# BraveenSri/siddhi

Hardware: AMD Instinct MI355X
Metric: events/sec (whole node) for partitioned pattern query at 1/2/4/8 GPUs; % HBM peak (higher is better)
Workload: dtype f32

## Files before the change

### siddhi_amd/csrc/gwalk.h

```cpp
#pragma once
#include <hip/hip_runtime.h>

#include <algorithm>
#include <cstdlib>
#include <cstring>
#include <type_traits>

#include "keypart.h"
#include "sg_engine.h"
#include "sg_prim.h"
#include "walk.h"

struct GwArgs {
  int64_t n, nc;
  int64_t within;
  int64_t t0;
  uint32_t K, ns1;
  int32_t stack_mode;
  int32_t cap;
  int32_t chunk;
  int32_t carry_out;
  int32_t pzero;
  const uint32_t* o1;
  const PtU4* grec;
  const uint8_t* glk;
  const uint32_t* kbase;
  uint64_t* trig;
  uint64_t* area;
  int64_t* cv_ts;
  int32_t* cv_key;
  int64_t* cv_val;
  int64_t* cv_pay;
  uint32_t* cv_n;
  uint32_t cv_cap;
  uint32_t* flags;
  uint32_t* ovf_keys;
  uint32_t* ovf_n;
  uint32_t ovf_cap;
  uint32_t* match_n;
};
static const uint32_t GW_ORDER = 1, GW_OVERFLOW = 2, GW_INTERNAL = 4, GW_CARRY_FULL = 8;

static __global__ void __launch_bounds__(256) k_gw_count(const uint32_t* __restrict__ o1, uint32_t ns1, uint32_t K,
                                                         const uint8_t* __restrict__ glk, uint32_t* __restrict__ kcnt) {
  __shared__ uint32_t c[4][256];
  const uint32_t g = blockIdx.x, t = threadIdx.x, w = t >> 6;
#pragma unroll
  for (int q = 0; q < 4; ++q) c[q][t] = 0;
  __syncthreads();
  const uint32_t lo = o1[(size_t)g * ns1], hi = o1[(size_t)(g + 1) * ns1];
  for (uint32_t p = lo + t; p < hi; p += 256) atomicAdd(&c[w][glk[p]], 1u);
  __syncthreads();
  const uint32_t k = (g << 8) + t;
  if (k < K) kcnt[k] = c[0][t] + c[1][t] + c[2][t] + c[3][t];
}

template <int PT>
struct GwLds {
  PtU4 stage[256 * PT];
  uint32_t cw[4][256];
  uint32_t ls[256], tot[256];
  uint32_t wsum[4];
};

template <class T>
struct GwLdsRing {
  T* v;
  int32_t* t;
  int32_t* p;
  uint32_t cmask, lane;
  __device__ __forceinline__ uint32_t ix(uint32_t s) const { return (s & cmask) * 256 + lane; }
  __device__ __forceinline__ bool full(uint32_t head, uint32_t top) const { return top - head == cmask + 1; }
};
template <class T>
struct GwHbmRing {
  T* v;
  int32_t* t;
  int32_t* p;
  __device__ __forceinline__ uint32_t ix(uint32_t s) const { return s; }
  __device__ __forceinline__ bool full(uint32_t, uint32_t) const { return false; }
};

template <class T, int OP, bool STACK, class RING>
struct GwLane {
  RING R;
  uint32_t head = 0, top = 0;
  int32_t hts = 0, prev = INT32_MIN;
  T tv = T();
  bool bad = false;
  uint64_t cur = 0;
  uint32_t k = 0;
  uint32_t nm = 0;
  uint32_t wi = 0;
  __device__ __forceinline__ bool step(const GwArgs& a, const PtU4& q) {
    const int32_t dts = (int32_t)q.x;
    const uint32_t rowf = q.y;
    T x;
    const uint32_t xb = q.z;
    __builtin_memcpy(&x, &xb, sizeof(T));
    const int32_t pay = (int32_t)q.w;
    const uint32_t f = rowf >> 30;
    bad |= dts < prev;
    prev = dts;
    if (!f) return true;
    const bool live = !is_nan_val<T>(x);
    if (head != top && (uint32_t)(dts - hts) > wi) {
      ++head;
      while (head != top) {
        hts = R.t[R.ix(head)];
        if ((uint32_t)(dts - hts) <= wi) break;
        ++head;
      }
    }
    const uint32_t r = rowf & ROW_MASK;
    uint32_t m = 0;
    if ((f & F_CONS) && live) {
      const bool emit = r >= (uint32_t)a.nc;
      const uint64_t hdr = cur;
      if constexpr (STACK) {
        if (top != head && cmp_op<T>(OP, x, tv)) {
          --top;
          ++m;
          while (top != head) {
            tv = R.v[R.ix(top - 1)];
            if (!cmp_op<T>(OP, x, tv)) break;
            --top;
            ++m;
          }
        }
        if (emit && m) {
          for (uint32_t e = 0; e < m; ++e) {
            const uint32_t s = R.ix(top + e);
            a.area[hdr + 2 + e] = (uint64_t)(uint32_t)val_bits<T>(R.v[s]) | ((uint64_t)(uint32_t)R.p[s] << 32);
          }
        }
      } else {
        uint32_t wr = head;
        for (uint32_t s = head; s != top; ++s) {
          const uint32_t si = R.ix(s);
          const T e = R.v[si];
          if (cmp_op<T>(OP, x, e)) {
            if (emit) a.area[hdr + 2 + m] = (uint64_t)(uint32_t)val_bits<T>(e) | ((uint64_t)(uint32_t)R.p[si] << 32);
            ++m;
          } else {
            if (wr != s) {
              const uint32_t wx = R.ix(wr);
              R.v[wx] = e;
              R.t[wx] = R.t[si];
              R.p[wx] = R.p[si];
            }
            ++wr;
          }
        }
        top = wr;
        if (head != top) {
          hts = R.t[R.ix(head)];
          tv = R.v[R.ix(top - 1)];
        }
      }
      if (emit && m) {
        const uint64_t b = r - (uint32_t)a.nc;
        a.area[hdr] = (uint64_t)(uint32_t)dts | ((uint64_t)k << 32);
        a.area[hdr + 1] = (uint64_t)(uint32_t)val_bits<T>(x) | ((uint64_t)(uint32_t)pay << 32);
        a.trig[b] = hdr | ((uint64_t)m << 32);
        cur = hdr + 2 + m;
        nm += m;
      }
    }
    if ((f & F_CAND) && live) {
      if (R.full(head, top)) return false;
      const uint32_t s = R.ix(top);
      R.v[s] = x;
      R.t[s] = dts;
      R.p[s] = pay;
      if (top == head) hts = dts;
      tv = x;
      ++top;
    }
    return true;
  }
  __device__ __forceinline__ void carry(const GwArgs& a, uint32_t o) const {
    for (uint32_t e = 0; e < top - head; ++e) {
      const uint32_t s = R.ix(head + e);
      a.cv_ts[o + e] = a.t0 + (int64_t)R.t[s];
      a.cv_key[o + e] = (int32_t)k;
      a.cv_val[o + e] = val_bits<T>(R.v[s]);
      a.cv_pay[o + e] = a.pzero ? (int64_t)(uint32_t)R.p[s] : (int64_t)R.p[s];
    }
  }
};

template <class T, int OP, int PT, bool STACK>
__global__ void __launch_bounds__(256, 1) k_gwalk(GwArgs a) {
  extern __shared__ __attribute__((aligned(16))) char lds_raw[];
  GwLds<PT>& L = *(GwLds<PT>*)lds_raw;
  const uint32_t cap = (uint32_t)a.cap;
  const uint32_t t = threadIdx.x, w = t >> 6, lane = t & 63;
  const uint32_t g = xcd_block(blockIdx.x, gridDim.x);
  const uint32_t k = (g << 8) + t;
  const bool active = k < a.K;
  const uint32_t lo = a.o1[(size_t)g * a.ns1], hi = a.o1[(size_t)(g + 1) * a.ns1];
  GwLane<T, OP, STACK, GwLdsRing<T>> W;
  W.R.v = (T*)(lds_raw + sizeof(GwLds<PT>));
  W.R.t = (int32_t*)(W.R.v + (size_t)cap * 256);
  W.R.p = W.R.t + (size_t)cap * 256;
  W.R.cmask = cap - 1;
  W.R.lane = t;
  W.k = k;
  W.wi = a.within > 0xffffffffll ? 0xffffffffu : (uint32_t)a.within;
  W.cur = active ? 3ull * a.kbase[k] : 0ull;
  bool ovf = false;
  const uint32_t ROWS = 256 * PT;
  PtU4 rc[PT], rn[PT];
  uint32_t tg[PT], tn[PT];
  auto load = [&](uint32_t base, PtU4* r, uint32_t* d) {
    const uint32_t rows = min(ROWS, hi - base);
#pragma unroll
    for (int s = 0; s < PT; ++s) {
      const uint32_t i = w * (PT * 64) + s * 64 + lane;
      const uint32_t p = base + (i < rows ? i : rows - 1);
      r[s] = __builtin_nontemporal_load(a.grec + p);
      d[s] = a.glk[p];
    }
  };
  if (lo < hi) load(lo, rc, tg);
  for (uint32_t base = lo; base < hi; base += ROWS) {
    {
      const uint32_t rows = min(ROWS, hi - base);
#pragma unroll
      for (int s = 0; s < PT; ++s)
        if (w * (PT * 64) + s * 64 + lane >= rows) tg[s] = 0xffffffffu;
    }
#pragma unroll
    for (int q = 0; q < 4; ++q) L.cw[q][t] = 0;
    __syncthreads();
#pragma unroll
    for (int s = 0; s < PT; ++s)
      if (tg[s] != 0xffffffffu) atomicAdd(&L.cw[w][tg[s]], 1u);
    __syncthreads();
    {
      const uint32_t c0 = L.cw[0][t], c1 = L.cw[1][t], c2 = L.cw[2][t], c3 = L.cw[3][t];
      const uint32_t tt = c0 + c1 + c2 + c3;
      const uint32_t ex = block_excl_scan256(tt, L.wsum);
      L.ls[t] = ex;
      L.tot[t] = tt;
      L.cw[0][t] = ex;
      L.cw[1][t] = ex + c0;
      L.cw[2][t] = ex + c0 + c1;
      L.cw[3][t] = ex + c0 + c1 + c2;
    }
    __syncthreads();
#pragma unroll
    for (int s = 0; s < PT; ++s) {
      const bool valid = tg[s] != 0xffffffffu;
      const uint32_t d = valid ? tg[s] : 0u;
      uint32_t rank, cnt;
      peer_rank(valid, d, 8, rank, cnt);
      if (valid) {
        const uint32_t slot = L.cw[w][d] + rank;
        if (rank == 0) L.cw[w][d] = slot + cnt;
        L.stage[slot] = rc[s];
      }
    }
    if (base + ROWS < hi) load(base + ROWS, rn, tn);
    __syncthreads();
    const uint32_t i0 = L.ls[t], i1 = i0 + L.tot[t];
    for (uint32_t i = i0; i < i1 && active && !ovf; ++i)
      if (!W.step(a, L.stage[i])) ovf = true;
    __syncthreads();
#pragma unroll
    for (int s = 0; s < PT; ++s) { rc[s] = rn[s]; tg[s] = tn[s]; }
  }
  uint32_t fl = W.bad ? GW_ORDER : 0u;
  if (active && W.cur > 3ull * a.kbase[k + 1]) fl |= GW_INTERNAL;
  if (ovf) {
    const uint32_t o = atomicAdd(a.ovf_n, 1u);
    if (o < a.ovf_cap) a.ovf_keys[o] = k;
    else fl |= GW_OVERFLOW;
  }
  if (fl) atomicOr(a.flags, fl);
  {
    uint32_t c = (active && !ovf) ? W.nm : 0u;
#pragma unroll
    for (int o = 32; o > 0; o >>= 1) c += (uint32_t)__shfl_xor((int)c, o);
    if (lane == 0 && c) atomicAdd(a.match_n, c);
  }
  if (!a.carry_out) return;
  const uint32_t m = (active && !ovf) ? W.top - W.head : 0u;
  uint32_t incl = m;
#pragma unroll
  for (int o = 1; o < 64; o <<= 1) {
    const uint32_t y = (uint32_t)__shfl_up((int)incl, o);
    if ((int)lane >= o) incl += y;
  }
  const uint32_t tot = (uint32_t)__shfl((int)incl, 63);
  if (!tot) return;
  uint32_t cb = 0;
  if (lane == 63) cb = atomicAdd(a.cv_n, tot);
  cb = (uint32_t)__shfl((int)cb, 63);
  if ((uint64_t)cb + tot > (uint64_t)a.cv_cap) {
    if (lane == 63) atomicOr(a.flags, GW_CARRY_FULL);
    return;
  }
  if (m) W.carry(a, cb + incl - m);
}

static const uint32_t GW_REDO_LDS = 2048;
template <class T, int OP, bool STACK>
__global__ void __launch_bounds__(256) k_gw_redo(GwArgs a, uint32_t* __restrict__ rows, T* __restrict__ hv,
                                                 int32_t* __restrict__ ht, int32_t* __restrict__ hp) {
  __shared__ uint32_t wc[4], base_s;
  __shared__ PtU4 red_stage[GW_REDO_LDS];
  __shared__ T red_v[GW_REDO_LDS];
  __shared__ int32_t red_t[GW_REDO_LDS], red_p[GW_REDO_LDS];
  const uint32_t k = a.ovf_keys[blockIdx.x];
  const uint32_t g = k >> 8, d = k & 255u, t = threadIdx.x, w = t >> 6, lane = t & 63;
  const uint32_t lo = a.o1[(size_t)g * a.ns1], hi = a.o1[(size_t)(g + 1) * a.ns1];
  const uint32_t kb = a.kbase[k], ke = a.kbase[k + 1];
  if (t == 0) base_s = 0;
  __syncthreads();
  for (uint32_t p0 = lo; p0 < hi; p0 += 256) {
    const uint32_t p = p0 + t;
    const bool mine = p < hi && a.glk[p] == d;
    const uint64_t bm = __ballot(mine);
    const uint32_t below = __builtin_amdgcn_mbcnt_hi((uint32_t)(bm >> 32), __builtin_amdgcn_mbcnt_lo((uint32_t)bm, 0u));
    if (lane == 0) wc[w] = (uint32_t)__popcll(bm);
    __syncthreads();
    uint32_t before = base_s;
    for (uint32_t q = 0; q < w; ++q) before += wc[q];
    if (mine && kb + before + below < ke) rows[kb + before + below] = p;
    __syncthreads();
    if (t == 0) base_s += wc[0] + wc[1] + wc[2] + wc[3];
    __syncthreads();
  }
  const uint32_t nk = ke - kb;
  const bool in_lds = nk <= GW_REDO_LDS;
  if (in_lds)
    for (uint32_t i = t; i < nk; i += 256) red_stage[i] = a.grec[rows[kb + i]];
  __syncthreads();
  if (t != 0) return;
  if (kb + base_s != ke) { atomicOr(a.flags, GW_INTERNAL); return; }
  GwLane<T, OP, STACK, GwHbmRing<T>> W;
  if (in_lds) {
    W.R.v = red_v;
    W.R.t = red_t;
    W.R.p = red_p;
  } else {
    W.R.v = hv + kb;
    W.R.t = ht + kb;
    W.R.p = hp + kb;
  }
  W.k = k;
  W.wi = a.within > 0xffffffffll ? 0xffffffffu : (uint32_t)a.within;
  W.cur = 3ull * kb;
  if (in_lds) for (uint32_t i = 0; i < nk; ++i) W.step(a, red_stage[i]);
  else for (uint32_t i = kb; i < ke; ++i) W.step(a, a.grec[rows[i]]);
  uint32_t fl = W.bad ? GW_ORDER : 0u;
  if (W.cur > 3ull * ke) fl |= GW_INTERNAL;
  if (fl) atomicOr(a.flags, fl);
  if (W.nm) atomicAdd(a.match_n, W.nm);
  if (!a.carry_out) return;
  const uint32_t m = W.top - W.head;
  if (!m) return;
  const uint32_t o = atomicAdd(a.cv_n, m);
  if ((uint64_t)o + m > (uint64_t)a.cv_cap) { atomicOr(a.flags, GW_CARRY_FULL); return; }
  W.carry(a, o);
}

struct GwSel {
  int32_t n_select, stride, multi, b_slot, pzero, vfloat;
  int32_t code[SG_MAX_SELECT];
};
static const int GW_PROJ_S = 256;
static const int GW_TILE = 256;

static __global__ void __launch_bounds__(256) k_gtile_count(int64_t n, const uint64_t* __restrict__ trig,
                                                            uint32_t* __restrict__ tcount, int64_t ntile) {
  __shared__ uint32_t red[8][4];
  const uint32_t t = threadIdx.x, w = t >> 6, lane = t & 63;
#pragma unroll
  for (int s = 0; s < 8; ++s) {
    const int64_t r = ((int64_t)blockIdx.x * 8 + s) * GW_TILE + t;
    uint32_t c = r < n ? (uint32_t)(__builtin_nontemporal_load(trig + r) >> 32) : 0u;
#pragma unroll
    for (int o = 32; o > 0; o >>= 1) c += (uint32_t)__shfl_xor((int)c, o);
    if (lane == 0) red[s][w] = c;
  }
  __syncthreads();
  if (t < 8) {
    const int64_t tile = (int64_t)blockIdx.x * 8 + t;
    if (tile < ntile) tcount[tile] = red[t][0] + red[t][1] + red[t][2] + red[t][3];
  }
}

static __global__ void __launch_bounds__(256) k_gscan_project(int64_t n, int64_t t0, uint64_t base_index,
                                                              const uint64_t* __restrict__ index,
                                                              const uint64_t* __restrict__ trig,
                                                              const uint64_t* __restrict__ area, GwSel sel,
                                                              int64_t out_base, char* __restrict__ out,
                                                              const uint32_t* __restrict__ tbase) {
  extern __shared__ __attribute__((aligned(16))) char stage[];
  __shared__ uint32_t wsum[4];
  const uint32_t t = threadIdx.x;
  const int64_t b = (int64_t)blockIdx.x * GW_TILE + t;
  const uint64_t tw = b < n ? __builtin_nontemporal_load(trig + b) : 0ull;
  const uint32_t m = (uint32_t)(tw >> 32);
  const uint64_t u = (uint32_t)tw;
  uint64_t h0 = 0, h1 = 0, tg = 0;
  if (m) {
    h0 = area[u];
    h1 = area[u + 1];
    tg = index ? index[b] : base_index + (uint64_t)b;
  }
  const uint32_t excl = block_excl_scan256(m, wsum);
  const uint32_t pre = tbase[blockIdx.x];
  const uint32_t o_lo = pre, o_hi = pre + (wsum[0] + wsum[1] + wsum[2] + wsum[3]);
  const uint32_t o = pre + excl;
  auto wid = [&](uint32_t bits, bool zero) { return zero ? (int64_t)bits : (int64_t)(int32_t)bits; };
  uint32_t nmask = 0;
  for (int s = 0; s < sel.n_select; ++s) nmask |= (sel.code[s] == 4) ? 1u << s : 0u;
  const int64_t ts = t0 + (int64_t)(int32_t)(uint32_t)h0;
  const uint32_t key = (uint32_t)(h0 >> 32);
  const int64_t v2 = wid((uint32_t)h1, sel.vfloat), p2 = wid((uint32_t)(h1 >> 32), sel.pzero);
  typedef uint32_t U4 __attribute__((ext_vector_type(4)));
  for (uint32_t sub = o_lo; sub < o_hi; sub += GW_PROJ_S) {
    const uint32_t se = (o_hi - sub < (uint32_t)GW_PROJ_S) ? o_hi : sub + GW_PROJ_S;
    if (m && o < se && o + m > sub) {
      const uint32_t qa = o < sub ? sub - o : 0u, qe = (o + m > se) ? se - o : m;
      for (uint32_t q = qa; q < qe; ++q) {
        const uint64_t e = area[u + 2 + q];
        const int64_t v1 = wid((uint32_t)e, sel.vfloat), p1 = wid((uint32_t)(e >> 32), sel.pzero);
        int64_t* r = (int64_t*)(stage + (size_t)(o + q - sub) * sel.stride);
        r[0] = (int64_t)tg;
        r[1] = ts;
        r[2] = (int64_t)((uint64_t)key | ((uint64_t)((1u << 24) | (sel.multi ? (uint32_t)sel.b_slot : (0x800000u | q))) << 32));
        r[3] = (int64_t)nmask;
        for (int c = 0; c < sel.n_select; ++c) {
          const int code = sel.code[c];
          r[4 + c] = code == 0 ? p1 : code == 1 ? v1 : code == 2 ? v2 : code == 3 ? p2 : 0;
        }
      }
    }
    __syncthreads();
    const size_t bytes = (size_t)(se - sub) * sel.stride;
    char* dst = out + (size_t)(out_base + sub) * sel.stride;
    if ((((uintptr_t)dst) & 15) == 0) {
      for (size_t x = (size_t)t * 16; x + 16 <= bytes; x += 256 * 16) *(U4*)(dst + x) = *(const U4*)(stage + x);
      if ((bytes & 8) && t == 255) *(uint64_t*)(dst + bytes - 8) = *(const uint64_t*)(stage + bytes - 8);
    } else {
      for (size_t x = (size_t)t * 8; x < bytes; x += 256 * 8) *(uint64_t*)(dst + x) = *(const uint64_t*)(stage + x);
    }
    __syncthreads();
  }
}

struct GwPlan {
  bool ok = false;
  int cap = 0;
  GwSel sel;
};
template <class T>
static GwPlan gw_plan(SgHandle* h, const BatchView& bv, int64_t n, int64_t nc, uint32_t kb, const PushPlan& plan,
                      bool same_col, int64_t span_ms) {
  const sg_nfa_desc& d = h->desc;
  GwPlan g;
  memset(&g.sel, 0, sizeof(g.sel));
  if (!d.partitioned || !same_col || plan.e1_row || d.n_select > SG_MAX_SELECT) return g;
  for (int c = 0; c < d.n_cols; ++c)
    if (bv.cols.nul[c]) return g;
  for (int s = 0; s < d.n_select; ++s) {
    const int src = plan.pp.src[s], kind = plan.pp.kind[s];
    int code = -1;
    if (kind == 2) code = 4;
    else if (kind == 0 && src == 0) code = 0;
    else if (kind == 1) code = src ? 2 : 1;
    else if (kind == 3 && src == 1 && plan.pcol >= 0 && plan.pp.col[s] == plan.pcol) code = 3;
    if (code < 0) return g;
    g.sel.code[s] = code;
  }
  const int64_t win = window_rows(kb, nc + n, d.within, span_ms);
  const char* e = getenv("SG_DEBUG_GW_CAP");
  int cap = h->opt.ring_cap > 0 ? h->opt.ring_cap : (e ? atoi(e) : pick_cap(win));
  if (cap > 32 || cap < 2 || (cap & (cap - 1))) return g;
  g.cap = cap;
  g.sel.n_select = d.n_select;
  g.sel.stride = 32 + 8 * d.n_select;
  g.sel.vfloat = std::is_same<T, float>::value ? 1 : 0;
  g.ok = true;
  return g;
}

template <class T, int OP, int PT, bool STACK>
static void launch_gwalk_pt(const GwArgs& ga, uint32_t ng, hipStream_t st) {
  const size_t lds = sizeof(GwLds<PT>) + (size_t)ga.cap * 256 * (sizeof(T) + 8);
  HIPCHK(hipFuncSetAttribute((const void*)k_gwalk<T, OP, PT, STACK>, hipFuncAttributeMaxDynamicSharedMemorySize, (int)lds));
  hipLaunchKernelGGL((k_gwalk<T, OP, PT, STACK>), dim3(ng), dim3(256), lds, st, ga);
  HIPCHK(hipGetLastError());
}
template <class T, int OP>
static void launch_gw_redo(const GwArgs& ga, uint32_t nk, uint32_t* rows, T* hv, int32_t* ht, int32_t* hp, hipStream_t st) {
  if (ga.stack_mode) hipLaunchKernelGGL((k_gw_redo<T, OP, true>), dim3(nk), dim3(256), 0, st, ga, rows, hv, ht, hp);
  else hipLaunchKernelGGL((k_gw_redo<T, OP, false>), dim3(nk), dim3(256), 0, st, ga, rows, hv, ht, hp);
  HIPCHK(hipGetLastError());
}
template <class T, int OP>
static void launch_gwalk(const GwArgs& ga, uint32_t ng, hipStream_t st) {
  const char* e = getenv("SG_DEBUG_GW_PT");
  const int pt = e ? atoi(e) : (ga.cap <= 8 ? 8 : ga.cap <= 16 ? 6 : 4);
  if (ga.stack_mode) {
    if (pt == 4) launch_gwalk_pt<T, OP, 4, true>(ga, ng, st);
    else if (pt == 12) launch_gwalk_pt<T, OP, 12, true>(ga, ng, st);
    else if (pt == 10) launch_gwalk_pt<T, OP, 10, true>(ga, ng, st);
    else if (pt == 6) launch_gwalk_pt<T, OP, 6, true>(ga, ng, st);
    else launch_gwalk_pt<T, OP, 8, true>(ga, ng, st);
  } else {
    launch_gwalk_pt<T, OP, 8, false>(ga, ng, st);
  }
}

static void gw_project(SgHandle* h, const BatchView& bv, int64_t n, const GwArgs& ga, const GwSel& sel, uint32_t total) {
  const sg_nfa_desc& d = h->desc;
  hipStream_t st = h->stream;
  char* out = h->out.reserve(total, d.n_select, st);
  const int64_t ntile = (n + GW_TILE - 1) / GW_TILE;
  uint32_t* tcount = (uint32_t*)h->ws.get("gw_tcount", sizeof(uint32_t) * ((size_t)ntile + 1), st);
  uint32_t* tbase = (uint32_t*)h->ws.get("gw_tbase", sizeof(uint32_t) * ((size_t)ntile + 1), st);
  h->kbeg("gw_tiles");
  HIPCHK(hipMemsetAsync(tcount + ntile, 0, sizeof(uint32_t), st));
  hipLaunchKernelGGL(k_gtile_count, dim3((unsigned)((ntile + 7) / 8)), dim3(256), 0, st, n, (const uint64_t*)ga.trig, tcount,
                     ntile);
  HIPCHK(hipGetLastError());
  sg_exclusive_scan(h->ws, st, "gw_tscan_tmp", tcount, tbase, (uint32_t)0, (size_t)ntile + 1, rocprim::plus<uint32_t>());
  h->kend();
  uint32_t tsum = 0;
  HIPCHK(hipMemcpyAsync(&tsum, tbase + ntile, sizeof(uint32_t), hipMemcpyDeviceToHost, st));
  h->kbeg("gw_project");
  const size_t plds = (size_t)GW_PROJ_S * sel.stride;
  if (plds > 65536)
    HIPCHK(hipFuncSetAttribute((const void*)k_gscan_project, hipFuncAttributeMaxDynamicSharedMemorySize, (int)plds));
  hipLaunchKernelGGL(k_gscan_project, dim3((unsigned)ntile), dim3(256), plds, st, n, ga.t0, bv.base_index, bv.index,
                     (const uint64_t*)ga.trig, (const uint64_t*)ga.area, sel, (int64_t)h->out.n, out,
                     (const uint32_t*)tbase);
  HIPCHK(hipGetLastError());
  h->kend();
  HIPCHK(hipStreamSynchronize(st));
  if (tsum != total) throw SgError(SG_EINVAL, "internal: group walker match count mismatch");
  h->out.n += total;
}

template <class T>
static int run_group_walk(SgHandle* h, const BatchView& bv, int64_t n, int64_t nc, uint32_t kb, const PartPlan& pp,
                          const uint32_t* o1, const WRec<T, true>* grec, const uint8_t* glk, uint32_t* pk_flags,
                          const GwPlan& gp, const PushPlan& plan, const Virt& v, const SgCols& cc, int op, int stack_mode,
                          int val_col_a, EveryNextState* es) {
  const sg_nfa_desc& d = h->desc;
  hipStream_t st = h->stream;
  const int64_t nt = nc + n;
  const uint32_t ng = (kb + 255) >> 8;
  uint32_t* kcnt = (uint32_t*)h->ws.get("gw_kcnt", sizeof(uint32_t) * ((size_t)kb + 1), st);
  uint32_t* kbase = (uint32_t*)h->ws.get("gw_kbase", sizeof(uint32_t) * ((size_t)kb + 1), st);
  h->kbeg("gw_count");
  HIPCHK(hipMemsetAsync(kcnt, 0, sizeof(uint32_t) * ((size_t)kb + 1), st));
  hipLaunchKernelGGL(k_gw_count, dim3(ng), dim3(256), 0, st, o1, pp.ns1, kb, glk, kcnt);
  HIPCHK(hipGetLastError());
  sg_exclusive_scan(h->ws, st, "gw_kscan_tmp", kcnt, kbase, (uint32_t)0, (size_t)kb + 1, rocprim::plus<uint32_t>());
  h->kend();
  uint32_t pkf = 0;
  int64_t t0 = 0;
  HIPCHK(hipMemcpyAsync(&pkf, pk_flags, sizeof(uint32_t), hipMemcpyDeviceToHost, st));
  HIPCHK(hipMemcpyAsync(&t0, nc ? v.c_ts : v.ts, sizeof(int64_t), hipMemcpyDeviceToHost, st));
  HIPCHK(hipStreamSynchronize(st));
  const PackRange pr = pack_range(pkf);
  if (pr == PACK_TS_RANGE) return 2;
  if (pr == PACK_PAY_RANGE) return 0;
  h->mark(2);

  GwArgs ga;
  memset(&ga, 0, sizeof(ga));
  ga.n = n;
  ga.nc = nc;
  ga.within = d.within;
  ga.t0 = t0;
  ga.K = kb;
  ga.ns1 = pp.ns1;
  ga.stack_mode = stack_mode;
  ga.cap = gp.cap;
  ga.chunk = 4096;
  ga.carry_out = h->opt.no_carry ? 0 : 1;
  ga.pzero = v.pfloat;
  ga.o1 = o1;
  ga.grec = (const PtU4*)grec;
  ga.glk = glk;
  ga.kbase = kbase;
  ga.trig = (uint64_t*)h->ws.get("gw_trig", sizeof(uint64_t) * ((size_t)n + 1), st);
  ga.area = (uint64_t*)h->ws.get("gw_area", sizeof(uint64_t) * 3 * (size_t)std::max<int64_t>(nt, 1), st);
  uint32_t* gflags = (uint32_t*)h->ws.get("gw_flags", sizeof(uint32_t) * 4, st);
  ga.flags = gflags;
  ga.cv_n = gflags + 1;
  ga.ovf_n = gflags + 2;
  ga.ovf_cap = std::min<uint32_t>(kb, 1u << 16);
  ga.ovf_keys = (uint32_t*)h->ws.get("gw_ovf_keys", sizeof(uint32_t) * ga.ovf_cap, st);
  ga.match_n = gflags + 3;
  ga.cv_cap = (uint32_t)std::max<int64_t>(1, std::min<int64_t>(nt, (int64_t)kb * gp.cap + (1 << 22)));
  ga.cv_ts = (int64_t*)h->ws.get("cv_ts", sizeof(int64_t) * (size_t)ga.cv_cap, st);
  ga.cv_val = (int64_t*)h->ws.get("cv_val", sizeof(int64_t) * (size_t)ga.cv_cap, st);
  ga.cv_pay = (int64_t*)h->ws.get("cv_pay", sizeof(int64_t) * (size_t)ga.cv_cap, st);
  ga.cv_key = (int32_t*)h->ws.get("cv_key", sizeof(int32_t) * (size_t)ga.cv_cap, st);
  HIPCHK(hipMemsetAsync(gflags, 0, sizeof(uint32_t) * 4, st));
  HIPCHK(hipMemsetAsync(ga.trig, 0, sizeof(uint64_t) * ((size_t)n + 1), st));
  h->kbeg("group_walk");
  dispatch_op(op, [&](auto opc) { launch_gwalk<T, decltype(opc)::value>(ga, ng, st); });
  h->kend();
  uint32_t hf[4] = {0, 0, 0, 0}, total = 0;
  HIPCHK(hipMemcpyAsync(hf, gflags, sizeof(hf), hipMemcpyDeviceToHost, st));
  HIPCHK(hipStreamSynchronize(st));
  if (hf[0] & GW_INTERNAL) throw SgError(SG_EINVAL, "internal: group walker guard tripped");
  if (hf[0]) return 0;
  if (hf[2]) {
    h->kbeg("gw_redo");
    uint32_t* rrows = (uint32_t*)h->ws.get("gw_redo_rows", sizeof(uint32_t) * (size_t)nt, st);
    char* rl = (char*)h->ws.get("gw_redo_list", (sizeof(T) + 8) * (size_t)nt, st);
    T* hv = (T*)rl;
    int32_t* ht = (int32_t*)(rl + sizeof(T) * (size_t)nt);
    int32_t* hp = ht + nt;
    dispatch_op(op, [&](auto opc) { launch_gw_redo<T, decltype(opc)::value>(ga, hf[2], rrows, hv, ht, hp, st); });
    h->kend();
    HIPCHK(hipMemcpyAsync(hf, gflags, sizeof(hf), hipMemcpyDeviceToHost, st));
    HIPCHK(hipStreamSynchronize(st));
    if (hf[0] & GW_INTERNAL) throw SgError(SG_EINVAL, "internal: group walker redo guard tripped");
    if (hf[0]) return 0;
  }
  h->last_spilled = hf[2];
  total = hf[3];
  h->mark(3);
  h->split_out = 1;
  h->mark(5);
  if (total) {
    GwSel sel = gp.sel;
    recv_slot(d, d.shape_args[1], sel.multi, sel.b_slot);
    sel.pzero = v.pfloat;
    gw_project(h, bv, n, ga, sel, total);
  }
  h->mark(4);
  if (ga.carry_out) {
    WalkArgs wa;
    memset(&wa, 0, sizeof(wa));
    wa.alive = (uint32_t*)h->ws.get("alive_rows", sizeof(uint32_t), st);
    wa.alive_n = (uint32_t*)h->ws.get("gw_alive_n", sizeof(uint32_t), st);
    HIPCHK(hipMemsetAsync(wa.alive_n, 0, sizeof(uint32_t), st));
    wa.cv_n = ga.cv_n;
    wa.cv_ts = ga.cv_ts;
    wa.cv_key = ga.cv_key;
    wa.cv_val = ga.cv_val;
    wa.cv_pay = ga.cv_pay;
    carry_out_rows<T, true>(h, es, nt, v, bv, cc, wa, val_col_a, v.pcol ? plan.pcol : -1, v.pw);
  }
  h->last_events = n;
  h->last_matches = total;
  return 1;
}
```

### siddhi_amd/csrc/sg_engine.h

```cpp
#pragma once
#include <hip/hip_runtime.h>

#include <algorithm>
#include <cstring>
#include <map>
#include <stdexcept>
#include <string>
#include <vector>

#include "../../include/siddhi_gpu.h"
#include "sg_device.h"

typedef sg_nfa_desc DevDesc;

struct SgError {
  int code;
  std::string msg;
  SgError(int c, std::string m) : code(c), msg(std::move(m)) {}
};

#define HIPCHK(x)                                                                                   \
  do {                                                                                              \
    hipError_t e_ = (x);                                                                            \
    if (e_ != hipSuccess) throw SgError(SG_EHIP, std::string(#x) + ": " + hipGetErrorString(e_)); \
  } while (0)

template <class T>
static T sg_read_back(const T* dp, hipStream_t st) {
  T v;
  HIPCHK(hipMemcpyAsync(&v, dp, sizeof(T), hipMemcpyDeviceToHost, st));
  HIPCHK(hipStreamSynchronize(st));
  return v;
}

struct Workspace {
  struct Buf { void* p = nullptr; size_t bytes = 0; };
  std::map<std::string, Buf> bufs;
  void* get(const std::string& name, size_t bytes, hipStream_t st) {
    Buf& b = bufs[name];
    if (bytes == 0) bytes = 16;
    if (b.bytes < bytes) {
      if (b.p) {
        hipStreamSynchronize(st);
        hipFree(b.p);
      }
      size_t want = bytes + bytes / 4;
      if (hipMalloc(&b.p, want) != hipSuccess) throw SgError(SG_EHIP, "hipMalloc failed for workspace " + name);
      b.bytes = want;
    }
    return b.p;
  }
  void release() {
    for (auto& kv : bufs) if (kv.second.p) hipFree(kv.second.p);
    bufs.clear();
  }
};

struct OutStore {
  int64_t n = 0, cap = 0;
  int nsel = 0;
  int stride = 32;
  char* rec = nullptr;
  char* reserve(int64_t extra, int n_select, hipStream_t st) {
    nsel = n_select;
    stride = 32 + 8 * n_select;
    int64_t need = n + extra;
    if (need > cap) {
      int64_t nc = std::max<int64_t>(need + need / 4, 1024);
      void* np = nullptr;
      if (hipMalloc(&np, (size_t)nc * stride) != hipSuccess) throw SgError(SG_EHIP, "hipMalloc failed for match store");
      if (rec && n) hipMemcpyAsync(np, rec, (size_t)n * stride, hipMemcpyDeviceToDevice, st);
      hipStreamSynchronize(st);
      if (rec) hipFree(rec);
      rec = (char*)np;
      cap = nc;
    }
    return rec;
  }
  void release() {
    if (rec) hipFree(rec);
    rec = nullptr;
    n = cap = 0;
  }
  void consume(int64_t k, hipStream_t st);
};

struct BatchView {
  int64_t n;
  uint64_t base_index;
  const int64_t* ts;
  const int32_t* stream;
  const int32_t* key;
  const uint64_t* index;
  SgCols cols;
  int32_t key_bound;
};

struct SgHandle {
  int device = 0;
  sg_nfa_desc desc;
  sg_options opt;
  DevDesc* ddesc = nullptr;
  hipStream_t stream = nullptr;
  bool own_stream = false;
  Workspace ws;
  OutStore out;
  OutStore stage;
  std::string err;
  hipEvent_t ev[8] = {};
  hipStream_t copy_stream = nullptr;
  hipEvent_t ev_copied[2] = {}, ev_consumed[2] = {};
  struct Egress {
    hipStream_t d2h = nullptr;
    char* stage[2] = {};
    int64_t cap[2] = {};
    hipEvent_t ready[2] = {}, done[2] = {};
  } eg;
  int64_t last_events = 0, last_matches = 0, last_spilled = 0;
  int pushes = 0;
  uint64_t gen = 0;
  std::vector<char> snap_cache;
  uint64_t snap_gen = ~0ull;
  uint32_t key_bound_seen = 0;
  int64_t ts_max_seen = INT64_MIN;
  void* state = nullptr;
  int state_kind = 0;
  int split_out = 0;
  int extra_marks = 0;
  void mark(int k) { hipEventRecord(ev[k], stream); }
  hipEvent_t km[SG_MAX_KMARKS][2] = {};
  const char* km_name[SG_MAX_KMARKS] = {};
  int n_km = 0;
  void kbeg(const char* name) {
    if (n_km >= SG_MAX_KMARKS) return;
    if (!km[n_km][0]) { hipEventCreate(&km[n_km][0]); hipEventCreate(&km[n_km][1]); }
    km_name[n_km] = name;
    hipEventRecord(km[n_km][0], stream);
  }
  void kend() {
    if (n_km >= SG_MAX_KMARKS) return;
    hipEventRecord(km[n_km][1], stream);
    ++n_km;
  }
  void bump_gen() {
    ++gen;
    if (!snap_cache.empty()) { std::vector<char>().swap(snap_cache); snap_gen = ~0ull; }
  }
};



struct SnapW {
  std::vector<char> b;
  void put(const void* p, size_t n) {
    size_t o = b.size();
    b.resize(o + n);
    if (n) memcpy(b.data() + o, p, n);
  }
  template <class T> void pod(const T& v) { put(&v, sizeof(T)); }
  void dev(const void* dp, size_t n, hipStream_t st) {
    size_t o = b.size();
    b.resize(o + n);
    if (!n) return;
    if (hipMemcpyAsync(b.data() + o, dp, n, hipMemcpyDeviceToHost, st) != hipSuccess || hipStreamSynchronize(st) != hipSuccess)
      throw SgError(SG_EHIP, "snapshot: device copy failed");
  }
};
struct SnapR {
  const char* p;
  const char* e;
  const char* take(size_t n) {
    if ((size_t)(e - p) < n) throw SgError(SG_EINVAL, "snapshot blob truncated");
    const char* q = p;
    p += n;
    return q;
  }
  template <class T> T pod() {
    T v;
    memcpy(&v, take(sizeof(T)), sizeof(T));
    return v;
  }
  void dev(void* dp, size_t n, hipStream_t st) {
    const char* q = take(n);
    if (!n) return;
    if (hipMemcpyAsync(dp, q, n, hipMemcpyHostToDevice, st) != hipSuccess || hipStreamSynchronize(st) != hipSuccess)
      throw SgError(SG_EHIP, "restore: device copy failed");
  }
};
void sg_every_next_snapshot(SgHandle* h, SnapW& w);
void sg_every_next_restore(SgHandle* h, SnapR& r);
void sg_every_absent_snapshot(SgHandle* h, SnapW& w);
void sg_every_absent_restore(SgHandle* h, SnapR& r);
void sg_general_snapshot(SgHandle* h, SnapW& w);
void sg_general_restore(SgHandle* h, SnapR& r);

struct SlotPtrs {
  void* ts = nullptr;
  void* stream = nullptr;
  void* key = nullptr;
  void* index = nullptr;
  void* col[SG_MAX_COLS] = {};
  void* nul[SG_MAX_COLS] = {};
};
struct ColLayout {
  int ns;
  int32_t width[SG_MAX_SELECT];
  size_t off_trig, off_ts, off_key, off_grp, off_col[SG_MAX_SELECT], off_nul[SG_MAX_SELECT], bytes;
};
int sg_col_width(int type);
SlotPtrs sg_reserve_slot(SgHandle& h, const sg_batch* b, int64_t rows, int slot);
BatchView sg_upload_to(const sg_nfa_desc& d, const SlotPtrs& p, const sg_batch* b, int64_t lo, int64_t cnt,
                       hipStream_t st);
void sg_push_view(SgHandle& h, BatchView& bv, int64_t n);
BatchView sg_slice_view(const sg_nfa_desc& d, const BatchView& bv, int64_t lo, int64_t cnt);
ColLayout sg_col_layout(const sg_nfa_desc& d, int64_t cap);
void sg_stage_reserve(SgHandle& h, int slot, int64_t bytes);
void sg_launch_to_columns(int64_t n, const char* rec, int stride, const ColLayout& L, char* stage, hipStream_t st);
void sg_egress_init(SgHandle& h);

void sg_run_every_next(SgHandle* h, const BatchView& bv, int64_t n);
void sg_every_next_f32(SgHandle* h, const BatchView& bv, int64_t n);
void sg_every_next_f64(SgHandle* h, const BatchView& bv, int64_t n);
void sg_every_next_i32(SgHandle* h, const BatchView& bv, int64_t n);
void sg_every_next_i64(SgHandle* h, const BatchView& bv, int64_t n);
void sg_every_next_reset(SgHandle* h);
void sg_every_next_release(SgHandle* h);
void sg_run_general(SgHandle* h, const BatchView& bv, int64_t n);
void sg_run_once(SgHandle* h, const BatchView& bv, int64_t n);
void sg_once_reset(SgHandle* h);
void sg_once_release(SgHandle* h);
void sg_once_snapshot(SgHandle* h, SnapW& w);
void sg_once_restore(SgHandle* h, SnapR& r);
void sg_run_every_absent(SgHandle* h, const BatchView& bv, int64_t n);
void sg_every_absent_reset(SgHandle* h);
void sg_every_absent_release(SgHandle* h);
void sg_general_reset(SgHandle* h);
void sg_general_release(SgHandle* h);
struct PartialState;
PartialState* sg_partial_new(const sg_nfa_desc& d);
void sg_partial_free(PartialState* ps);
void sg_partial_reset(PartialState* ps);
int sg_partial_active(const PartialState* ps);
void sg_partial_deactivate(PartialState* ps);
int sg_partial_push(SgHandle* h, PartialState* ps, const BatchView& bv, int64_t n, uint32_t key_bound);
int64_t sg_partial_max_rows(SgHandle* h, PartialState* ps);
int64_t sg_partial_carried(const PartialState* ps);
void sg_partial_snapshot(SgHandle* h, PartialState* ps, SnapW& w);
void sg_partial_restore(SgHandle* h, PartialState* ps, SnapR& r);
```

Measured before the change: 15.65 billion.

## Epoch-tag trigger words to skip per-batch memset of trigger buffer

Trigger words now carry an 8-bit epoch tag in their top bits, and readers treat words with a stale epoch as zero matches. This removes the per-batch memset of the n-entry trigger array; the buffer is cleared only when the epoch counter wraps or the buffer grows. Match counts are capped at 24 bits and larger counts raise an overflow flag. Select codes are also packed into 4-bit fields with a precomputed null mask, so the projection kernel no longer rebuilds the mask per thread.

After: 15.93 billion (median of 6 runs). No clear change (+1.8%).

```diff
diff --git a/siddhi_amd/csrc/gwalk.h b/siddhi_amd/csrc/gwalk.h
--- a/siddhi_amd/csrc/gwalk.h
+++ b/siddhi_amd/csrc/gwalk.h
@@ -26,6 +26,7 @@
   const uint8_t* glk;
   const uint32_t* kbase;
   uint64_t* trig;
+  uint32_t epoch;
   uint64_t* area;
   int64_t* cv_ts;
   int32_t* cv_key;
@@ -40,6 +41,14 @@
   uint32_t* match_n;
 };
 static const uint32_t GW_ORDER = 1, GW_OVERFLOW = 2, GW_INTERNAL = 4, GW_CARRY_FULL = 8;
+
+static const uint32_t GW_MATCH_MAX = (1u << 24) - 1;
+__device__ __forceinline__ uint64_t gw_trig_word(uint64_t unit, uint32_t m, uint32_t epoch) {
+  return unit | ((uint64_t)m << 32) | ((uint64_t)epoch << 56);
+}
+__device__ __forceinline__ uint32_t gw_trig_matches(uint64_t w, uint32_t epoch) {
+  return (uint32_t)(w >> 56) == epoch ? (uint32_t)(w >> 32) & GW_MATCH_MAX : 0u;
+}
 
 static __global__ void __launch_bounds__(256) k_gw_count(const uint32_t* __restrict__ o1, uint32_t ns1, uint32_t K,
                                                          const uint8_t* __restrict__ glk, uint32_t* __restrict__ kcnt) {
@@ -88,6 +97,7 @@
   int32_t hts = 0, prev = INT32_MIN;
   T tv = T();
   bool bad = false;
+  bool big = false;
   uint64_t cur = 0;
   uint32_t k = 0;
   uint32_t nm = 0;
@@ -162,7 +172,8 @@
         const uint64_t b = r - (uint32_t)a.nc;
         a.area[hdr] = (uint64_t)(uint32_t)dts | ((uint64_t)k << 32);
         a.area[hdr + 1] = (uint64_t)(uint32_t)val_bits<T>(x) | ((uint64_t)(uint32_t)pay << 32);
-        a.trig[b] = hdr | ((uint64_t)m << 32);
+        big |= m > GW_MATCH_MAX;
+        a.trig[b] = gw_trig_word(hdr, m & GW_MATCH_MAX, a.epoch);
         cur = hdr + 2 + m;
         nm += m;
       }
@@ -357,6 +368,7 @@
   else for (uint32_t i = kb; i < ke; ++i) W.step(a, a.grec[rows[i]]);
   uint32_t fl = W.bad ? GW_ORDER : 0u;
   if (W.cur > 3ull * ke) fl |= GW_INTERNAL;
+  if (W.big) fl |= GW_OVERFLOW;
   if (fl) atomicOr(a.flags, fl);
   if (W.nm) atomicAdd(a.match_n, W.nm);
   if (!a.carry_out) return;
@@ -369,19 +381,22 @@
 
 struct GwSel {
   int32_t n_select, stride, multi, b_slot, pzero, vfloat;
-  int32_t code[SG_MAX_SELECT];
+  uint32_t nmask;
+  uint32_t pad;
+  uint64_t codes[2];
 };
+static_assert(SG_MAX_SELECT <= 32, "GwSel packs 32 select codes");
 static const int GW_PROJ_S = 256;
 static const int GW_TILE = 256;
 
-static __global__ void __launch_bounds__(256) k_gtile_count(int64_t n, const uint64_t* __restrict__ trig,
+static __global__ void __launch_bounds__(256) k_gtile_count(int64_t n, const uint64_t* __restrict__ trig, uint32_t epoch,
                                                             uint32_t* __restrict__ tcount, int64_t ntile) {
   __shared__ uint32_t red[8][4];
   const uint32_t t = threadIdx.x, w = t >> 6, lane = t & 63;
 #pragma unroll
   for (int s = 0; s < 8; ++s) {
     const int64_t r = ((int64_t)blockIdx.x * 8 + s) * GW_TILE + t;
-    uint32_t c = r < n ? (uint32_t)(__builtin_nontemporal_load(trig + r) >> 32) : 0u;
+    uint32_t c = r < n ? gw_trig_matches(__builtin_nontemporal_load(trig + r), epoch) : 0u;
 #pragma unroll
     for (int o = 32; o > 0; o >>= 1) c += (uint32_t)__shfl_xor((int)c, o);
     if (lane == 0) red[s][w] = c;
@@ -395,7 +410,7 @@
 
 static __global__ void __launch_bounds__(256) k_gscan_project(int64_t n, int64_t t0, uint64_t base_index,
                                                               const uint64_t* __restrict__ index,
-                                                              const uint64_t* __restrict__ trig,
+                                                              const uint64_t* __restrict__ trig, uint32_t epoch,
                                                               const uint64_t* __restrict__ area, GwSel sel,
                                                               int64_t out_base, char* __restrict__ out,
                                                               const uint32_t* __restrict__ tbase) {
@@ -404,7 +419,7 @@
   const uint32_t t = threadIdx.x;
   const int64_t b = (int64_t)blockIdx.x * GW_TILE + t;
   const uint64_t tw = b < n ? __builtin_nontemporal_load(trig + b) : 0ull;
-  const uint32_t m = (uint32_t)(tw >> 32);
+  const uint32_t m = gw_trig_matches(tw, epoch);
   const uint64_t u = (uint32_t)tw;
   uint64_t h0 = 0, h1 = 0, tg = 0;
   if (m) {
@@ -417,8 +432,9 @@
   const uint32_t o_lo = pre, o_hi = pre + (wsum[0] + wsum[1] + wsum[2] + wsum[3]);
   const uint32_t o = pre + excl;
   auto wid = [&](uint32_t bits, bool zero) { return zero ? (int64_t)bits : (int64_t)(int32_t)bits; };
-  uint32_t nmask = 0;
-  for (int s = 0; s < sel.n_select; ++s) nmask |= (sel.code[s] == 4) ? 1u << s : 0u;
+  const uint64_t cw0 = sel.codes[0], cw1 = sel.codes[1];
+  const int nsel = sel.n_select;
+  const int64_t nmask = (int64_t)sel.nmask;
   const int64_t ts = t0 + (int64_t)(int32_t)(uint32_t)h0;
   const uint32_t key = (uint32_t)(h0 >> 32);
   const int64_t v2 = wid((uint32_t)h1, sel.vfloat), p2 = wid((uint32_t)(h1 >> 32), sel.pzero);
@@ -434,9 +450,9 @@
         r[0] = (int64_t)tg;
         r[1] = ts;
         r[2] = (int64_t)((uint64_t)key | ((uint64_t)((1u << 24) | (sel.multi ? (uint32_t)sel.b_slot : (0x800000u | q))) << 32));
-        r[3] = (int64_t)nmask;
-        for (int c = 0; c < sel.n_select; ++c) {
-          const int code = sel.code[c];
+        r[3] = nmask;
+        for (int c = 0; c < nsel; ++c) {
+          const uint32_t code = (uint32_t)((c < 16 ? cw0 >> (4 * c) : cw1 >> (4 * (c - 16))) & 15u);
           r[4 + c] = code == 0 ? p1 : code == 1 ? v1 : code == 2 ? v2 : code == 3 ? p2 : 0;
         }
       }
@@ -476,7 +492,8 @@
     else if (kind == 1) code = src ? 2 : 1;
     else if (kind == 3 && src == 1 && plan.pcol >= 0 && plan.pp.col[s] == plan.pcol) code = 3;
     if (code < 0) return g;
-    g.sel.code[s] = code;
+    g.sel.codes[s >> 4] |= (uint64_t)code << (4 * (s & 15));
+    if (code == 4) g.sel.nmask |= 1u << s;
   }
   const int64_t win = window_rows(kb, nc + n, d.within, span_ms);
   const char* e = getenv("SG_DEBUG_GW_CAP");
@@ -518,6 +535,23 @@
   }
 }
 
+static uint64_t* gw_tagged_words(SgHandle* h, SgHandle::GwTagged& tw, const char* name, size_t words, bool wrap,
+                                 hipStream_t st) {
+  uint64_t* p = (uint64_t*)h->ws.get(name, sizeof(uint64_t) * words, st);
+  const size_t cap = h->ws.bufs[name].bytes;
+  if (p != tw.p || cap != tw.cap) {
+    tw.p = p;
+    tw.cap = cap;
+    tw.hw = 0;
+  }
+  if (wrap && tw.hw) HIPCHK(hipMemsetAsync(p, 0, sizeof(uint64_t) * tw.hw, st));
+  if (words > tw.hw) {
+    HIPCHK(hipMemsetAsync(p + tw.hw, 0, sizeof(uint64_t) * (words - tw.hw), st));
+    tw.hw = words;
+  }
+  return p;
+}
+
 static void gw_project(SgHandle* h, const BatchView& bv, int64_t n, const GwArgs& ga, const GwSel& sel, uint32_t total) {
   const sg_nfa_desc& d = h->desc;
   hipStream_t st = h->stream;
@@ -527,8 +561,8 @@
   uint32_t* tbase = (uint32_t*)h->ws.get("gw_tbase", sizeof(uint32_t) * ((size_t)ntile + 1), st);
   h->kbeg("gw_tiles");
   HIPCHK(hipMemsetAsync(tcount + ntile, 0, sizeof(uint32_t), st));
-  hipLaunchKernelGGL(k_gtile_count, dim3((unsigned)((ntile + 7) / 8)), dim3(256), 0, st, n, (const uint64_t*)ga.trig, tcount,
-                     ntile);
+  hipLaunchKernelGGL(k_gtile_count, dim3((unsigned)((ntile + 7) / 8)), dim3(256), 0, st, n, (const uint64_t*)ga.trig, ga.epoch,
+                     tcount, ntile);
   HIPCHK(hipGetLastError());
   sg_exclusive_scan(h->ws, st, "gw_tscan_tmp", tcount, tbase, (uint32_t)0, (size_t)ntile + 1, rocprim::plus<uint32_t>());
   h->kend();
@@ -539,7 +573,7 @@
   if (plds > 65536)
     HIPCHK(hipFuncSetAttribute((const void*)k_gscan_project, hipFuncAttributeMaxDynamicSharedMemorySize, (int)plds));
   hipLaunchKernelGGL(k_gscan_project, dim3((unsigned)ntile), dim3(256), plds, st, n, ga.t0, bv.base_index, bv.index,
-                     (const uint64_t*)ga.trig, (const uint64_t*)ga.area, sel, (int64_t)h->out.n, out,
+                     (const uint64_t*)ga.trig, ga.epoch, (const uint64_t*)ga.area, sel, (int64_t)h->out.n, out,
                      (const uint32_t*)tbase);
   HIPCHK(hipGetLastError());
   h->kend();
@@ -592,7 +626,12 @@
   ga.grec = (const PtU4*)grec;
   ga.glk = glk;
   ga.kbase = kbase;
-  ga.trig = (uint64_t*)h->ws.get("gw_trig", sizeof(uint64_t) * ((size_t)n + 1), st);
+  const char* ee = getenv("SG_DEBUG_GW_EPOCHS");
+  const uint32_t epochs = ee ? (uint32_t)std::min(std::max(atoi(ee), 1), 255) : 255u;
+  const bool wrap = h->gw_epoch >= epochs;
+  h->gw_epoch = wrap ? 1u : h->gw_epoch + 1;
+  ga.epoch = h->gw_epoch;
+  ga.trig = gw_tagged_words(h, h->gw_trig, "gw_trig", (size_t)std::max<int64_t>(n, 1), wrap, st);
   ga.area = (uint64_t*)h->ws.get("gw_area", sizeof(uint64_t) * 3 * (size_t)std::max<int64_t>(nt, 1), st);
   uint32_t* gflags = (uint32_t*)h->ws.get("gw_flags", sizeof(uint32_t) * 4, st);
   ga.flags = gflags;
@@ -607,7 +646,6 @@
   ga.cv_pay = (int64_t*)h->ws.get("cv_pay", sizeof(int64_t) * (size_t)ga.cv_cap, st);
   ga.cv_key = (int32_t*)h->ws.get("cv_key", sizeof(int32_t) * (size_t)ga.cv_cap, st);
   HIPCHK(hipMemsetAsync(gflags, 0, sizeof(uint32_t) * 4, st));
-  HIPCHK(hipMemsetAsync(ga.trig, 0, sizeof(uint64_t) * ((size_t)n + 1), st));
   h->kbeg("group_walk");
   dispatch_op(op, [&](auto opc) { launch_gwalk<T, decltype(opc)::value>(ga, ng, st); });
   h->kend();
diff --git a/siddhi_amd/csrc/sg_engine.h b/siddhi_amd/csrc/sg_engine.h
--- a/siddhi_amd/csrc/sg_engine.h
+++ b/siddhi_amd/csrc/sg_engine.h
@@ -123,6 +123,9 @@
   uint64_t snap_gen = ~0ull;
   uint32_t key_bound_seen = 0;
   int64_t ts_max_seen = INT64_MIN;
+  struct GwTagged { const void* p = nullptr; size_t cap = 0, hw = 0; };
+  GwTagged gw_trig;
+  uint32_t gw_epoch = 0;
   void* state = nullptr;
   int state_kind = 0;
   int split_out = 0;
```
